# AgamChopra/TorchRegister

Hardware: AMD Instinct MI355X
Metric: registration iterations/sec (3D 256^3 fp32, affine+NCC) (higher is better)
Workload: dtype f32; 1 GPU; 3D 256^3 fp32 affine+NCC, 8 independent pairs per GPU (BASELINE.json configs[3] share of one GPU), ADAM on theta; pairs_per_gpu=8, pairs_total=8, loss=NCC(alpha=100), optimizer=adam, preconditioning=100 untimed iterations before the warm-up (clock settling); value_cold has none, parallelism=1 x independent shards, no collective

## Files before the change

### include/trx.h

```cpp
#ifndef TRX_H
#define TRX_H

#include <stddef.h>
#include <stdint.h>

#ifdef __cplusplus
extern "C" {
#endif

#define TRX_VERSION 240
#define TRX_PSTRIDE 12

typedef enum {
    TRX_OK = 0,
    TRX_ERR_ARG = -1,
    TRX_ERR_NDIM = -2,
    TRX_ERR_WORKSPACE = -3,
    TRX_ERR_HIP = -4,
    TRX_ERR_CAPACITY = -5
} trx_status;

#define TRX_FLAG_GATHER_PATH 1u
#define TRX_FLAG_SINGLE_GEOM 2u
#define TRX_FLAG_TWO_PASS_FLOW 4u
// ... 8 lines not shown
#define TRX_FLAG_WALK_DOWN 8192u
#define TRX_FLAG_NO_PINGPONG 16384u
#define TRX_FLAG_NO_ZS_FLAT 4096u
#define TRX_FLAG_ONE_KERNEL 32768u
#define TRX_FLAG_NO_CARRY 65536u
#define TRX_FLAG_NO_ROT_DEEP_TILE 16u

typedef struct {
    const float *moving;
    const float *target;
    size_t moving_stride;
    size_t target_stride;
    int ndim, B, D, H, W;
    const float *xn, *yn, *zn;
    unsigned flags;
} trx_volumes;

typedef struct {
    float w_mse, w_ncc, ncc_alpha, w_ssd, ssd_alpha;
} trx_loss_cfg;

typedef enum { TRX_OPT_SGD = 0, TRX_OPT_ADAM = 1 } trx_opt_kind;
typedef struct {
    int kind;
    float lr, beta1, beta2, eps;
} trx_opt_cfg;

typedef enum { TRX_PARAM_AFFINE = 0, TRX_PARAM_RIGID = 1 } trx_param_mode;

typedef struct {
    int mode;
    float *param;
    float *theta;
    float *adam_m;
    float *adam_v;
    float *best_theta;
    float *best_loss;
    int *best_idx;
    float *losses;
    int losses_capacity;
    int *step;
    float *grad;
} trx_affine_state;

int trx_version(void);
const char *trx_status_string(int status);

size_t trx_affine_workspace_bytes(const trx_volumes *vol );

size_t trx_affine_workspace_rows_offset(const trx_volumes *vol );

int trx_affine_near_identity(const trx_volumes *vol , const float *theta_host);

int trx_affine_step(const trx_volumes *vol, const trx_loss_cfg *loss, const trx_opt_cfg *opt,
                    const trx_affine_state *st, void *workspace, size_t workspace_bytes, void *stream);

int trx_affine_accumulate(const trx_volumes *vol, const float *theta, void *workspace, size_t workspace_bytes, void *stream);

int trx_affine_run(const trx_volumes *vol, const trx_loss_cfg *loss, const trx_opt_cfg *opt,
                   const trx_affine_state *st, int iters, void *workspace, size_t workspace_bytes, void *stream);

int trx_affine_loss(const trx_volumes *vol, const trx_loss_cfg *loss, const float *theta, float *terms,
                    void *workspace, size_t workspace_bytes, void *stream);

int trx_affine_warp(const trx_volumes *vol, const float *theta, int channels, float *out, void *stream);

int trx_affine_warp_backward(const trx_volumes *vol, const float *theta, int channels, const float *grad_out,
                             float *dtheta, void *workspace, size_t workspace_bytes, void *stream);

int trx_affine_warp_lattice(const trx_volumes *vol, const float *theta, const int *iz, int nz, const int *iy, int ny, const int *ix, int nx,
                            float *out, void *stream);
int trx_affine_warp_lattice_backward(const trx_volumes *vol, const float *theta, const int *iz, int nz, const int *iy, int ny, const int *ix,
                                     int nx, const float *grad_out, float *dtheta, void *workspace, size_t workspace_bytes, void *stream);

int trx_theta_chain(const float *pose, const float *dtheta, int ndim, int B, float *theta_out, float *dpose_out, void *stream);

typedef struct {
    float *flow;
    float *flow_tmp;
    float *adam_m;
    float *adam_v;
    float *losses;
    int losses_capacity;
    int *step;
    float smooth_weight;
    float stop_crit;
    int *stopped;
    float *flow_last;
} trx_flow_state;

size_t trx_flow_workspace_bytes(const trx_volumes *vol);

int trx_flow_warp(const trx_volumes *vol, const float *flow, int channels, float *out, void *stream);

int trx_flow_step(const trx_volumes *vol, const trx_loss_cfg *loss, const trx_opt_cfg *opt,
                  const trx_flow_state *st, void *workspace, size_t workspace_bytes, void *stream);
int trx_flow_run(const trx_volumes *vol, const trx_loss_cfg *loss, const trx_opt_cfg *opt,
                 const trx_flow_state *st, int iters, void *workspace, size_t workspace_bytes, void *stream);

int trx_flow_loss_grad(const trx_volumes *vol, const trx_loss_cfg *loss, const float *flow, float *terms,
                       float *dflow, void *workspace, size_t workspace_bytes, void *stream);

int trx_flow_slab_moments(const trx_volumes *vol, int z_offset, int D_full, const float *flow, int smooth, const float *halo_hi, double *moments,
                          void *workspace, size_t workspace_bytes, void *stream);
int trx_flow_slab_update(const trx_volumes *vol, int z_offset, int D_full, const trx_loss_cfg *loss, const trx_opt_cfg *opt,
                         const trx_flow_state *st, const double *global_moments, const float *halo_lo, const float *halo_hi,
// ... 64 lines not shown
```

### torchregister_amd/_lib.py

```python
import ctypes
import os

import torch

_HERE = os.path.dirname(os.path.abspath(__file__))
LIB_PATH = os.path.join(_HERE, "lib", "libtrx.so")

PSTRIDE = 12
OPT_SGD, OPT_ADAM = 0, 1
PARAM_AFFINE, PARAM_RIGID = 0, 1
FLAG_GATHER_PATH, FLAG_SINGLE_GEOM, FLAG_TWO_PASS_FLOW, FLAG_DEEP_TILE, FLAG_NO_ROT_DEEP_TILE, FLAG_NO_ZSTREAM, FLAG_ZSTREAM, FLAG_NEAREST, FLAG_SAVE_LAST = 1, 2, 4, 8, 16, 32, 64, 128, 256
FLAG_NO_EFT, FLAG_EFT = 512, 1024
FLAG_WALK_DOWN, FLAG_NO_PINGPONG = 8192, 16384
FLAG_NO_ZS_FLAT = 4096
FLAG_ONE_KERNEL = 32768
FLAG_NO_CARRY = 65536
FLAG_ZS_FUSED = 2048

c_float_p = ctypes.POINTER(ctypes.c_float)
c_int_p = ctypes.POINTER(ctypes.c_int)


class TrxError(RuntimeError):
    pass


class Volumes(ctypes.Structure):
    _fields_ = [("moving", ctypes.c_void_p), ("target", ctypes.c_void_p),
                ("moving_stride", ctypes.c_size_t), ("target_stride", ctypes.c_size_t),
                ("ndim", ctypes.c_int), ("B", ctypes.c_int), ("D", ctypes.c_int), ("H", ctypes.c_int), ("W", ctypes.c_int),
                ("xn", ctypes.c_void_p), ("yn", ctypes.c_void_p), ("zn", ctypes.c_void_p), ("flags", ctypes.c_uint)]


class LossCfg(ctypes.Structure):
    _fields_ = [("w_mse", ctypes.c_float), ("w_ncc", ctypes.c_float), ("ncc_alpha", ctypes.c_float),
                ("w_ssd", ctypes.c_float), ("ssd_alpha", ctypes.c_float)]


class OptCfg(ctypes.Structure):
    _fields_ = [("kind", ctypes.c_int), ("lr", ctypes.c_float), ("beta1", ctypes.c_float), ("beta2", ctypes.c_float),
                ("eps", ctypes.c_float)]


class AffineState(ctypes.Structure):
    _fields_ = [("mode", ctypes.c_int), ("param", ctypes.c_void_p), ("theta", ctypes.c_void_p),
                ("adam_m", ctypes.c_void_p), ("adam_v", ctypes.c_void_p), ("best_theta", ctypes.c_void_p),
                ("best_loss", ctypes.c_void_p), ("best_idx", ctypes.c_void_p), ("losses", ctypes.c_void_p),
                ("losses_capacity", ctypes.c_int), ("step", ctypes.c_void_p), ("grad", ctypes.c_void_p)]


class FlowState(ctypes.Structure):
    _fields_ = [("flow", ctypes.c_void_p), ("flow_tmp", ctypes.c_void_p), ("adam_m", ctypes.c_void_p),
                ("adam_v", ctypes.c_void_p), ("losses", ctypes.c_void_p), ("losses_capacity", ctypes.c_int),
                ("step", ctypes.c_void_p), ("smooth_weight", ctypes.c_float), ("stop_crit", ctypes.c_float),
                ("stopped", ctypes.c_void_p), ("flow_last", ctypes.c_void_p)]


_P = ctypes.c_void_p
SIGNATURES = {
    "trx_version": (ctypes.c_int, []),
    "trx_status_string": (ctypes.c_char_p, [ctypes.c_int]),
    "trx_affine_workspace_bytes": (ctypes.c_size_t, [ctypes.POINTER(Volumes)]),
    "trx_affine_workspace_rows_offset": (ctypes.c_size_t, [ctypes.POINTER(Volumes)]),
    "trx_affine_near_identity": (ctypes.c_int, [ctypes.POINTER(Volumes), _P]),
    "trx_affine_step": (ctypes.c_int, [ctypes.POINTER(Volumes), ctypes.POINTER(LossCfg), ctypes.POINTER(OptCfg),
                                       ctypes.POINTER(AffineState), _P, ctypes.c_size_t, _P]),
    "trx_affine_accumulate": (ctypes.c_int, [ctypes.POINTER(Volumes), _P, _P, ctypes.c_size_t, _P]),
    "trx_affine_run": (ctypes.c_int, [ctypes.POINTER(Volumes), ctypes.POINTER(LossCfg), ctypes.POINTER(OptCfg),
                                      ctypes.POINTER(AffineState), ctypes.c_int, _P, ctypes.c_size_t, _P]),
    "trx_affine_loss": (ctypes.c_int, [ctypes.POINTER(Volumes), ctypes.POINTER(LossCfg), _P, _P, _P, ctypes.c_size_t, _P]),
    "trx_affine_warp": (ctypes.c_int, [ctypes.POINTER(Volumes), _P, ctypes.c_int, _P, _P]),
    "trx_affine_warp_backward": (ctypes.c_int, [ctypes.POINTER(Volumes), _P, ctypes.c_int, _P, _P, _P, ctypes.c_size_t, _P]),
    "trx_theta_chain": (ctypes.c_int, [_P, _P, ctypes.c_int, ctypes.c_int, _P, _P, _P]),
    "trx_affine_warp_lattice": (ctypes.c_int, [ctypes.POINTER(Volumes), _P, _P, ctypes.c_int, _P, ctypes.c_int, _P, ctypes.c_int, _P, _P]),
    "trx_affine_warp_lattice_backward": (ctypes.c_int, [ctypes.POINTER(Volumes), _P, _P, ctypes.c_int, _P, ctypes.c_int, _P, ctypes.c_int, _P, _P, _P,
                                                        ctypes.c_size_t, _P]),
    "trx_flow_workspace_bytes": (ctypes.c_size_t, [ctypes.POINTER(Volumes)]),
    "trx_flow_warp": (ctypes.c_int, [ctypes.POINTER(Volumes), _P, ctypes.c_int, _P, _P]),
    "trx_flow_step": (ctypes.c_int, [ctypes.POINTER(Volumes), ctypes.POINTER(LossCfg), ctypes.POINTER(OptCfg),
                                     ctypes.POINTER(FlowState), _P, ctypes.c_size_t, _P]),
    "trx_flow_run": (ctypes.c_int, [ctypes.POINTER(Volumes), ctypes.POINTER(LossCfg), ctypes.POINTER(OptCfg),
                                    ctypes.POINTER(FlowState), ctypes.c_int, _P, ctypes.c_size_t, _P]),
    "trx_flow_slab_moments": (ctypes.c_int, [ctypes.POINTER(Volumes), ctypes.c_int, ctypes.c_int, _P, ctypes.c_int, _P, _P, _P, ctypes.c_size_t, _P]),
    "trx_flow_slab_boundary_smooth": (ctypes.c_int, [ctypes.POINTER(Volumes), _P, _P, _P, _P]),
    "trx_peer_signal": (ctypes.c_int, [_P, ctypes.c_uint, _P]),
    "trx_peer_wait": (ctypes.c_int, [_P, ctypes.c_uint, ctypes.c_uint, _P, _P]),
    "trx_peer_publish": (ctypes.c_int, [_P, _P, _P, ctypes.c_int, ctypes.c_uint, _P]),
    "trx_peer_gather": (ctypes.c_int, [_P, _P, ctypes.c_int, ctypes.c_uint, ctypes.c_uint, _P, _P, _P]),
    "trx_peer_alloc": (ctypes.c_int, [ctypes.c_size_t, ctypes.POINTER(ctypes.c_void_p)]),
    "trx_peer_free": (ctypes.c_int, [_P]),
    "trx_peer_export": (ctypes.c_int, [_P, _P]),
    "trx_peer_import": (ctypes.c_int, [_P, ctypes.POINTER(ctypes.c_void_p)]),
    "trx_peer_close": (ctypes.c_int, [_P]),
    "trx_flow_slab_update": (ctypes.c_int, [ctypes.POINTER(Volumes), ctypes.c_int, ctypes.c_int, ctypes.POINTER(LossCfg),
                                            ctypes.POINTER(OptCfg), ctypes.POINTER(FlowState), _P, _P, _P, _P, ctypes.c_size_t, _P]),
    "trx_flow_slab_update_fused": (ctypes.c_int, [ctypes.POINTER(Volumes), ctypes.c_int, ctypes.c_int, ctypes.POINTER(LossCfg),
                                                  ctypes.POINTER(OptCfg), ctypes.POINTER(FlowState), _P, _P, ctypes.c_size_t, _P]),
    "trx_flow_slab_moments_ready": (ctypes.c_int, [ctypes.POINTER(Volumes), ctypes.c_int, ctypes.c_int, _P, _P, ctypes.c_size_t, _P]),
    "trx_flow_loss_grad": (ctypes.c_int, [ctypes.POINTER(Volumes), ctypes.POINTER(LossCfg), _P, _P, _P, _P, ctypes.c_size_t, _P]),
    "trx_flow_warp_backward": (ctypes.c_int, [ctypes.POINTER(Volumes), _P, ctypes.c_int, _P, _P, _P]),
    "trx_kde_workspace_bytes": (ctypes.c_size_t, [ctypes.c_int, ctypes.c_long, ctypes.c_int]),
    "trx_kde_pdf": (ctypes.c_int, [_P, _P, ctypes.c_int, ctypes.c_long, ctypes.c_int, ctypes.c_float, _P, _P, ctypes.c_size_t, _P]),
    "trx_kde_pdf_backward": (ctypes.c_int, [_P, _P, _P, ctypes.c_int, ctypes.c_long, ctypes.c_int, ctypes.c_float, _P, _P]),
    "trx_kde_series_workspace_bytes": (ctypes.c_size_t, [ctypes.c_int, ctypes.c_long, ctypes.c_int]),
    "trx_kde_pdf_series": (ctypes.c_int, [_P, _P, ctypes.c_int, ctypes.c_long, ctypes.c_int, ctypes.c_float, ctypes.c_double, _P, _P, ctypes.c_size_t, _P]),
    "trx_kde_pdf_series_backward": (ctypes.c_int, [_P, _P, _P, ctypes.c_int, ctypes.c_long, ctypes.c_int, ctypes.c_float, ctypes.c_double, _P, _P,
                                                   ctypes.c_size_t, _P]),
    "trx_kde_pdf_series_cached": (ctypes.c_int, [_P, _P, ctypes.c_int, ctypes.c_int, ctypes.c_long, ctypes.c_int, ctypes.c_float, ctypes.c_double, _P, _P]),
    "trx_nmi_from_pdfs_pooled": (ctypes.c_int, [_P, _P, _P, ctypes.c_int, ctypes.c_int, ctypes.c_float, _P, _P, _P, _P, _P]),
    "trx_nmi_lattice_lines": (ctypes.c_int, [ctypes.POINTER(Volumes), _P, _P, ctypes.c_int, _P, ctypes.c_int, _P, ctypes.c_int, _P, _P, ctypes.c_int,
                                             ctypes.c_int, _P, _P, _P, ctypes.c_size_t, _P]),
    "trx_nmi_loop_update": (ctypes.c_int, [ctypes.c_int, _P, _P, _P, _P, ctypes.c_float, _P, ctypes.c_int, _P, _P, _P, _P, _P]),
    "trx_nmi_from_pdfs": (ctypes.c_int, [_P, _P, _P, ctypes.c_int, ctypes.c_int, ctypes.c_float, _P, _P, _P, _P, _P, _P, _P]),
    "trx_flow_lncc_workspace_bytes": (ctypes.c_size_t, [ctypes.POINTER(Volumes)]),
    "trx_flow_lncc_run": (ctypes.c_int, [ctypes.POINTER(Volumes), ctypes.c_int, ctypes.c_float, ctypes.c_float, ctypes.POINTER(OptCfg),
                                         ctypes.POINTER(FlowState), ctypes.c_int, _P, ctypes.c_size_t, _P]),
    "trx_lncc_workspace_bytes": (ctypes.c_size_t, [ctypes.c_int] * 5),
# ... 37 lines not shown
```

### torchregister_amd/csrc/affine.hip

```cpp
#ifdef TRX_DEV
#include <cstdlib>
#endif
#include "trx_dev.h"

#include "trx_common.h"

namespace trx {

struct AffineGeom {
    int TX, TY, logTX, RPT, nxseg, nychunk, nblk;
};

static AffineGeom affine_geom(const trx_volumes &v, int target_blocks_total)
{
    AffineGeom g;
    int tx = 16, l = 4;
    while (tx < v.W && tx < TRX_BLOCK) { tx <<= 1; l++; }
    g.TX = tx; g.logTX = l; g.TY = TRX_BLOCK / tx;
    g.nxseg = (v.W + tx - 1) / tx;
    long rows = (long)v.D * v.H * g.nxseg * v.B;
    long rpt = rows / ((long)g.TY * target_blocks_total);
    if (rpt < 1) rpt = 1;
    if (rpt > 64) rpt = 64;
    g.RPT = (int)rpt;
// ... 2061 lines not shown
    p.zs_first = p.flat && p.zg.blocks_per_pair > 0 && !(v.flags & TRX_FLAG_ZS_FUSED);
    p.one_kernel = p.zs_first && (v.flags & TRX_FLAG_ONE_KERNEL);
    const bool two_body = !p.flat && p.td.blocks_per_pair == 0 && p.trd.blocks_per_pair == 0 && p.zg.blocks_per_pair == 0 && p.eft == 0;
    p.dual = p.zs_first ? kBehindZs : !two_body ? kFiveBody : carry ? kCarry : kTwoBody;
    return p;
}

struct AffineWs {
    size_t rows, off_tab, off_rows_used, off_part2, off_rows_used2, off_carry, bytes;
};
static AffineWs affine_ws(const trx_volumes &v)
{
    AffineWs w;
    AffineGeom g = affine_geom(v, kTargetBlocks);
    w.rows = (size_t)g.nblk;
    if (v.ndim == 3) w.rows = max(w.rows, (size_t)f1_rows(f1_candidates(v)));
    w.off_tab = ((size_t)v.B * w.rows * np_full(3) * sizeof(float) + 255) & ~(size_t)255;
    w.off_rows_used = w.off_tab + (((size_t)(v.W + v.H + v.D) * sizeof(float) + 255) & ~(size_t)255);
    const size_t notes = ((size_t)(v.B + 11) * sizeof(int) + 255) & ~(size_t)255;
    w.off_part2 = w.off_rows_used + notes;
    w.off_rows_used2 = w.off_part2 + (v.ndim == 3 ? w.off_tab : 0);
    w.off_carry = w.off_rows_used2 + (v.ndim == 3 ? notes : 0);
    w.bytes = w.off_carry + (v.ndim == 3 ? (((size_t)2 * v.B * kCarryStride * sizeof(float) + 255) & ~(size_t)255) : 0);
    return w;
}

extern "C" size_t trx_affine_workspace_bytes(const trx_volumes *vol)
{
    if (check_vol(vol, false) != TRX_OK) return 0;
    return affine_ws(*vol).bytes;
}

extern "C" size_t trx_affine_workspace_rows_offset(const trx_volumes *vol)
{
    if (check_vol(vol, false) != TRX_OK) return 0;
    return affine_ws(*vol).off_rows_used;
}

extern "C" int trx_affine_near_identity(const trx_volumes *vol, const float *theta_host)
{
    if (check_vol(vol, false) != TRX_OK || !theta_host || vol->ndim != 3) return 0;
    const F1Plan p = f1_plan(*vol, persistent_blocks(), true, false);
    if (p.zg.blocks_per_pair == 0) return 0;
    const float fD = (float)vol->D, fH = (float)vol->H, fW = (float)vol->W;
    for (int b = 0; b < vol->B; b++) {
        const float *th = theta_host + (size_t)b * TRX_PSTRIDE;
        if (zs_nsub<ZS64>(th, fD, fH, fW, p.zg.planes_per_seg) > 0) continue;
        if (p.zgf.blocks_per_pair > 0 && zs_nsub<ZSF>(th, fD, fH, fW, p.zgf.planes_per_seg) > 0) continue;
        return 0;
    }
    return 1;
}

static bool use_tile_path(const trx_volumes *vol) { return vol->ndim == 3 && !(vol->flags & TRX_FLAG_GATHER_PATH); }

struct CarryLaunch {
    int parity;
    CarryKArgs args;
    bool used;
    float *partials_out;
};

template <int MODE>
static int launch_accum(const trx_volumes *vol, const float *theta, const AffineGeom &g, int channels, size_t chan_stride,
                        float *partials, hipStream_t s)
{
    dim3 grid(g.nblk, vol->B), block(TRX_BLOCK);
    if (vol->ndim == 3)
        hipLaunchKernelGGL((affine_accum_kernel<3, MODE>), grid, block, 0, s, *vol, theta, g, channels, chan_stride, partials);
    else
        hipLaunchKernelGGL((affine_accum_kernel<2, MODE>), grid, block, 0, s, *vol, theta, g, channels, chan_stride, partials);
    TRX_CHECK_LAUNCH();
    return TRX_OK;
}

template <int MODE>
static void launch_dual(const F1Plan &p, hipStream_t s, const trx_volumes &v, const float *theta, int channels, float *out, int *rows_used = nullptr,
                        const CarryKArgs *carry = nullptr)
{
    const dim3 grid = p.flat ? dim3(p.slots, 1) : dim3(p.rows, v.B * channels);
    const int zero_surplus = rows_used == nullptr, rows_stride = p.flat ? p.rows : 0;
    auto launch = [&](auto which, auto... carry_args) {
        hipLaunchKernelGGL((affine_tile_dual_kernel<MODE, decltype(which)::value>), grid, dim3(512), 0, s, v, theta, p.ta, p.tr, channels, out, zero_surplus, p.td, p.trd, p.zg,
                           rows_used, rows_stride, p.eft, carry_args...);
    };
    if constexpr (MODE == 0 || MODE == 4)
        if (p.dual == kCarry) return launch(Which<kCarry>{}, *carry);
    if constexpr (MODE == 0 || MODE == 1 || MODE == 4)
        if (p.dual == kBehindZs) return launch(Which<kBehindZs>{});
    p.dual == kTwoBody ? launch(Which<kTwoBody>{}) : launch(Which<kFiveBody>{});
}

template <int MODE>
static int launch_f1(const trx_volumes *vol, const float *theta, float *partials, int *nblk, hipStream_t s, const int **rows_used = nullptr, CarryLaunch *cl = nullptr)
{
    if (rows_used) *rows_used = nullptr;
    if (cl) cl->used = false;
    if (!use_tile_path(vol)) {
        if constexpr (MODE == 4) return TRX_ERR_ARG;
        else {
            AffineGeom g = affine_geom(*vol, kTargetBlocks);
            *nblk = g.nblk;
            return launch_accum<MODE>(vol, theta, g, 1, 0, partials, s);
        }
    }
    trx_volumes v = *vol;
// ... 353 lines not shown
```

### torchregister_amd/csrc/affine_zstream.h

```cpp

#ifndef TRX_ZS_DBG
#define TRX_ZS_DBG 0
#endif
#ifndef TRX_ZS_MIN_WAVES
#define TRX_ZS_MIN_WAVES 4
#endif
#ifndef TRX_ZS_PRIO_BIT
#define TRX_ZS_PRIO_BIT 14
#endif
#ifndef TRX_ZS_STAMP
#define TRX_ZS_STAMP 0
#endif
#if TRX_ZS_STAMP
__device__ unsigned long long trx_zs_stamps[512 * 8 * 8];
#endif

struct ZAcc {
    f2 Axy[3], Bxy[3], ABz[3], M01, M23;
    float M4;
};
__device__ __forceinline__ unsigned long long sgpr_pair(float lo, float hi)
{
    const unsigned l = (unsigned)__builtin_amdgcn_readfirstlane(__float_as_int(lo)), h = (unsigned)__builtin_amdgcn_readfirstlane(__float_as_int(hi));
    return ((unsigned long long)h << 32) | l;
}
__device__ __forceinline__ void zs_lerp_accumulate(f2 r00, f2 r01, f2 r10, f2 r11, float tx, float ty, float tz, float yv, float yn, unsigned long long yn2, ZAcc &a)
{
    const f2 dz0 = r10 - r00, dz1 = r11 - r01;
    const f2 z0 = dz0 * tz + r00, z1 = dz1 * tz + r01;
    const f2 dy = z1 - z0;
    const f2 vv = dy * ty + z0;
    const f2 dzy = (dz1 - dz0) * ty + dz0;
    f2 yw, gxy, gz2;
    yw.x = yv;
    gxy.x = vv.y - vv.x;
    asm("v_fma_f32 %0, %1, %2, %3" : "=v"(yw.y) : "v"(tx), "v"(gxy.x), "v"(vv.x));
    asm("v_fma_f32 %0, %1, %2, %3" : "=v"(gxy.y) : "v"(tx), "v"(dy.y - dy.x), "v"(dy.x));
    asm("v_fma_f32 %0, %1, %2, %3" : "=v"(gz2.x) : "v"(tx), "v"(dzy.y - dzy.x), "v"(dzy.x));
    gz2.y = yn * gz2.x;
    f2 ygxy;
    asm("v_pk_mul_f32 %0, %1, %2" : "=v"(ygxy) : "v"(gxy), "s"(yn2));
    a.M01 += yw;
    a.M23 = yw * yw + a.M23;
    a.M4 = fmaf(yw.x, yw.y, a.M4);
    a.Axy[0] += gxy; a.Bxy[0] += ygxy; a.ABz[0] += gz2;
    a.Axy[1] = gxy * yw.x + a.Axy[1]; a.Bxy[1] = ygxy * yw.x + a.Bxy[1]; a.ABz[1] = gz2 * yw.x + a.ABz[1];
    a.Axy[2] = gxy * yw.y + a.Axy[2]; a.Bxy[2] = ygxy * yw.y + a.Bxy[2]; a.ABz[2] = gz2 * yw.y + a.ABz[2];
}

template <int TX_, int TY_, int NZ_, int BW_, int BH_>
struct ZCfg {
    static constexpr int TX = TX_, TY = TY_, NZ = NZ_, BW = BW_, BH = BH_;
    static constexpr int Threads = 512, Waves = 8;
    static constexpr int XW = TX / 64, RG = Waves / XW, R = TY / RG;
    static constexpr int BW4 = BW / 4, PlaneSlots = BH * BW4;
    static constexpr int LPP = (PlaneSlots + 15) / 16;
    static constexpr int PlaneFloats = BW * BH, PlaneBytes = PlaneFloats * 4;
    static constexpr int RingFloats = NZ * PlaneFloats;
    static constexpr int Lead = 1;
    static constexpr int Span = NZ - Lead;
    static constexpr int ReduceScratch = Waves * 16 * 65 + Waves * 16;
    static constexpr int Alloc = (RingFloats + 4 > ReduceScratch) ? RingFloats + 4 : ReduceScratch;
    static_assert(TX % 64 == 0 && Waves % XW == 0 && TY % RG == 0 && BW % 4 == 0 && LPP <= 64 && NZ >= 4 && NZ <= 8 && Span <= 7, "geometry");
};
using ZSF = ZCfg<64, 16, 8, 80, 30>;
using ZS64 = ZCfg<64, 32, 7, 72, 40>;

struct ZGeom {
    int ntx, nty, nzseg, planes_per_seg, blocks_per_pair;
};

template <class C>
static ZGeom zs_geom(const trx_volumes &v)
{
    ZGeom g;
    g.ntx = v.W / C::TX; g.nty = v.H / C::TY;
    const long cols = (long)v.B * g.ntx * g.nty;
    int nseg = cols >= 512 ? 1 : (int)((512 + cols - 1) / cols);
    const int cap = v.D / 32 > 1 ? v.D / 32 : 1;
    if (nseg > cap) nseg = cap;
    g.planes_per_seg = (v.D + nseg - 1) / nseg;
    g.nzseg = (v.D + g.planes_per_seg - 1) / g.planes_per_seg;
    g.blocks_per_pair = g.ntx * g.nty * g.nzseg;
    return g;
}

template <class C>
static bool zs_shape_ok(const trx_volumes &v)
{
    if (v.ndim != 3 || v.W % C::TX || v.H % C::TY || v.D < 8) return false;
    return (size_t)v.D * v.H * v.W < ((size_t)1 << 29);
}

template <class C>
__host__ __device__ __forceinline__ bool zs_fits_len(const float *__restrict__ th, float fD, float fH, float fW, int len)
{
    const float ex = (float)(C::TX - 1), ey = (float)(C::TY - 1), ez = (float)(len - 1);
    const float sx = fabsf(th[0]) * ex + fabsf(th[1] * fW / fH) * ey + fabsf(th[2] * fW / fD) * ez;
    const float sy = fabsf(th[4] * fH / fW) * ex + fabsf(th[5]) * ey + fabsf(th[6] * fH / fD) * ez;
    const float sz = fabsf(th[8] * fD / fW) * ex + fabsf(th[9] * fD / fH) * ey + fabsf(th[10] - 1.0f) * ez;
    return (sx <= (float)C::BW - 6.3f) && (sy <= (float)C::BH - 3.3f) && (sz <= (float)C::Span - 3.3f);
}
template <class C>
__host__ __device__ __forceinline__ int zs_nsub(const float *__restrict__ th, float fD, float fH, float fW, int planes_per_seg)
{
    if (zs_fits_len<C>(th, fD, fH, fW, planes_per_seg)) return 1;
    if (planes_per_seg >= 64 && zs_fits_len<C>(th, fD, fH, fW, (planes_per_seg + 1) / 2)) return 2;
    if (planes_per_seg >= 128 && zs_fits_len<C>(th, fD, fH, fW, (planes_per_seg + 3) / 4)) return 4;
    if (planes_per_seg >= 128 && zs_fits_len<C>(th, fD, fH, fW, (planes_per_seg + 7) / 8)) return 8;
    return 0;
}

#pragma clang diagnostic push
#pragma clang diagnostic ignored "-Winline-asm"
#pragma clang diagnostic ignored "-Wint-to-pointer-cast"
template <int MODE, class C>
__device__ __forceinline__ void zstream_body(const trx_volumes &vol, const float *__restrict__ theta, const ZGeom &zg, float *__restrict__ partials,
                                             float *ring, const int bx, const int by, int rows_per_pair, const int wave_in, const int second_slot = 0)
{
    const int walk_down = __builtin_amdgcn_readfirstlane((int)(vol.flags & TRX_FLAG_WALK_DOWN));
    const int dir = walk_down ? -1 : 1;
    const bool down = walk_down != 0;
    static_assert(MODE == 0 || MODE == 1 || MODE == 4, "step kernels and the moments pass");
    constexpr int NQ = (MODE == 0) ? 3 : (MODE == 4 ? 1 : 0);
    constexpr int NP = (MODE == 0) ? np_full(3) : (MODE == 4 ? kNpMse : 5);
    constexpr bool kGrad = MODE != 1;
    constexpr int R = C::R;
    const int b = by;
    const int D = vol.D, H = vol.H, W = vol.W;
    const float *__restrict__ th = uni_ptr(theta + (size_t)b * TRX_PSTRIDE);
    const float *__restrict__ mov = uni_ptr(vol.moving + (size_t)b * vol.moving_stride);
    const float *__restrict__ tgt = uni_ptr(vol.target + (size_t)b * vol.target_stride);
    const float *__restrict__ xtab = uni_ptr(vol.xn), *__restrict__ ytab = uni_ptr(vol.yn), *__restrict__ ztab = uni_ptr(vol.zn);
    const int lane = trx_lane_id();
    const int wave = __builtin_amdgcn_readfirstlane(wave_in);
    const int tid = wave * 64 + lane;
    const float fW = (float)W, fH = (float)H, fD = (float)D;
    const float hW = 0.5f * fW, hH = 0.5f * fH, hD = 0.5f * fD;
    const float t00 = th[0], t01 = th[1], t02 = th[2], t03 = th[3];
    const float t10 = th[4], t11 = th[5], t12 = th[6], t13 = th[7];
    const float t20 = th[8], t21 = th[9], t22 = th[10], t23 = th[11];

    const int ncol = zg.ntx * zg.nty, nblk = zg.blocks_per_pair;
    int lb = bx;
    if ((nblk & 7) == 0) lb = (bx & 7) * (nblk >> 3) + (bx >> 3);
    const int zseg = lb / ncol, col = lb - zseg * ncol;
    const int X0 = (col % zg.ntx) * C::TX, Y0 = (col / zg.ntx) * C::TY;
    const int zb0 = zseg * zg.planes_per_seg, ze0 = min(zb0 + zg.planes_per_seg, D);
    const int nsub = max(1, __builtin_amdgcn_readfirstlane(zs_nsub<C>(th, fD, fH, fW, zg.planes_per_seg)));
    const int sublen = (zg.planes_per_seg + nsub - 1) / nsub;

    const int xw = wave % C::XW, rg = wave / C::XW;
    const int x = X0 + xw * 64 + lane, yrow0 = Y0 + rg * R;
    const float xn = xtab[x];
    const float cx = unnorm<3>(xn, fW) + hW * fmaf(t00 - 1.0f, xn, t03);
    const float cy = hH * fmaf(t10, xn, t13);
    const float cz = hD * fmaf(t20, xn, t23);
    const float kxz = uni(hW * t02), kyz = uni(hH * t12), kzz = uni(hD * (t22 - 1.0f));
    float yn_r[R], sx_r[R], ey_r[R], sz_r[R];
#pragma unroll
    for (int j = 0; j < R; j++) {
        const float yn = ytab[yrow0 + j];
        yn_r[j] = uni(yn);
        sx_r[j] = uni((hW * t01) * yn);
        ey_r[j] = uni(unnorm<3>(yn, fH) + (hH * (t11 - 1.0f)) * yn);
        sz_r[j] = uni((hD * t21) * yn);
    }
    constexpr bool kV2 = MODE == 0 && (R % 2 == 0);
    unsigned long long sx2[(R + 1) / 2], ey2[(R + 1) / 2], sz2[(R + 1) / 2], yn2[R];
    if constexpr (kV2) {
#pragma unroll
        for (int k = 0; k < R / 2; k++) {
            sx2[k] = sgpr_pair(sx_r[2 * k], sx_r[2 * k + 1]);
            ey2[k] = sgpr_pair(ey_r[2 * k], ey_r[2 * k + 1]);
            sz2[k] = sgpr_pair(sz_r[2 * k], sz_r[2 * k + 1]);
        }
#pragma unroll
        for (int j = 0; j < R; j++) yn2[j] = sgpr_pair(yn_r[j], yn_r[j]);
    }
    auto coord = [&](int xi, int yi, int zi, float &ix, float &iy, float &iz) {
        const float a = xtab[xi], bb = ytab[yi], c = ztab[zi];
        ix = unnorm<3>(a, fW) + hW * fmaf(t00 - 1.0f, a, fmaf(t01, bb, fmaf(t02, c, t03)));
        iy = unnorm<3>(bb, fH) + hH * fmaf(t10, a, fmaf(t11 - 1.0f, bb, fmaf(t12, c, t13)));
        iz = unnorm<3>(c, fD) + hD * fmaf(t20, a, fmaf(t21, bb, fmaf(t22 - 1.0f, c, t23)));
    };

    const unsigned ring_lds = (unsigned)(uintptr_t)ring;
    const unsigned dummy_lds = ring_lds + C::RingFloats * 4u;
    const unsigned pl0 = ring_lds + (unsigned)(wave * C::LPP * 16), pl1 = ring_lds + (unsigned)((wave + 8) * C::LPP * 16);
    const size_t plane_bytes = (size_t)H * W * 4;
    const unsigned toffb = (unsigned)((yrow0 * W) + x) * 4u;
    int ys_s, ps_s;
    asm("s_mov_b32 %0, %1" : "=s"(ys_s) : "i"(C::BW * 4));
    asm("s_mov_b32 %0, %1" : "=s"(ps_s) : "i"(C::PlaneBytes));
    typedef const __attribute__((address_space(3))) f2u *lds_f2;

    F1Acc acc;
#pragma unroll
    for (int q = 0; q < 3; q++)
#pragma unroll
        for (int c = 0; c < 3; c++) acc.AB[q][c] = (f2)(0.f);
    acc.M01 = acc.M23 = (f2)(0.f);
    acc.M4 = 0.f;
    ZAcc acc2;
    f2 Uxy[3];
    float Uz[3];
#pragma unroll
    for (int q = 0; q < 3; q++) {
        acc2.Axy[q] = acc2.Bxy[q] = acc2.ABz[q] = Uxy[q] = (f2)(0.f);
        Uz[q] = 0.f;
    }
    acc2.M01 = acc2.M23 = (f2)(0.f);
    acc2.M4 = 0.f;
    float U[3][3];
#pragma unroll
    for (int q = 0; q < 3; q++)
#pragma unroll
        for (int c = 0; c < 3; c++) U[q][c] = 0.f;
    bool ok = true;
#if TRX_ZS_STAMP
    unsigned long long stamp_sum[6] = {0, 0, 0, 0, 0, 0};
    const unsigned long long stamp_t0 = __builtin_amdgcn_s_memtime(), stamp_r0 = __builtin_amdgcn_s_memrealtime();
#endif

    for (int si = 0; si < nsub; si++) {
        const int sub = down ? nsub - 1 - si : si;
        const int zb = zb0 + sub * sublen, ze = min(zb + sublen, ze0);
        if (zb >= ze) continue;
        const int nsteps = ze - zb, last = nsteps - 1;
        const int zf = down ? ze - 1 : zb, zl = down ? zb : ze - 1;
        float mnx = 1e30f, mxx = -1e30f, mny = 1e30f, mxy = -1e30f, mnz0 = 1e30f, mxz0 = -1e30f, mnz1 = 1e30f, mxz1 = -1e30f;
#pragma unroll
        for (int k = 0; k < 8; k++) {
            float ix, iy, iz;
            coord(X0 + ((k & 1) ? C::TX - 1 : 0), Y0 + ((k & 2) ? C::TY - 1 : 0), (k & 4) ? zl : zf, ix, iy, iz);
            mnx = fminf(mnx, ix); mxx = fmaxf(mxx, ix); mny = fminf(mny, iy); mxy = fmaxf(mxy, iy);
            if (k & 4) { mnz1 = fminf(mnz1, iz); mxz1 = fmaxf(mxz1, iz); } else { mnz0 = fminf(mnz0, iz); mxz0 = fmaxf(mxz0, iz); }
        }
        const float slack = 0.05f;
        bool fits = (fabsf(mnx) < 1.0e6f) && (fabsf(mxx) < 1.0e6f) && (fabsf(mny) < 1.0e6f) && (fabsf(mxy) < 1.0e6f) && (fabsf(mnz0) < 1.0e6f) &&
                    (fabsf(mxz0) < 1.0e6f) && (fabsf(mnz1) < 1.0e6f) && (fabsf(mxz1) < 1.0e6f);
        int ox = 0, oy = 0, pbase = 0, need_rows = 0, need_c4 = 0;
        if (fits) {
            ox = (int)floorf(mnx - slack) & ~3;
            oy = (int)floorf(mny - slack);
            const int hx = (int)floorf(mxx + slack) + 1, hy = (int)floorf(mxy + slack) + 1;
            need_rows = hy - oy; need_c4 = (hx - ox) >> 2;
            const int hi0 = (int)floorf(mxz0 + slack) + 1, hi1 = (int)floorf(mxz1 + slack) + 1;
            const int lo0 = (int)floorf(mnz0 - slack), lo1 = (int)floorf(mnz1 - slack);
            if (!down) {
                pbase = max(hi0, hi1 - last);
                fits = (hx <= ox + C::BW - 1) && (hy <= oy + C::BH - 1) && (lo0 >= pbase - (C::Span - 1)) && (lo1 >= pbase + last - (C::Span - 1));
            } else {
                pbase = min(lo0, lo1 + last);
                fits = (hx <= ox + C::BW - 1) && (hy <= oy + C::BH - 1) && (hi0 <= pbase + (C::Span - 1)) && (hi1 <= pbase - last + (C::Span - 1));
            }
        }
        ox = __builtin_amdgcn_readfirstlane(ox); oy = __builtin_amdgcn_readfirstlane(oy); pbase = __builtin_amdgcn_readfirstlane(pbase);
        need_rows = __builtin_amdgcn_readfirstlane(need_rows); need_c4 = __builtin_amdgcn_readfirstlane(need_c4);
        if (!__builtin_amdgcn_readfirstlane((int)fits)) { ok = false; break; }

        for (int i = tid; i < C::RingFloats / 4; i += C::Threads) reinterpret_cast<float4 *>(ring)[i] = make_float4(0.f, 0.f, 0.f, 0.f);
        unsigned long long mk[2];
        unsigned voff[2];
        bool pvalid[2];
#pragma unroll
        for (int k = 0; k < 2; k++) {
            const int q = wave + 8 * k;
            const int slot = q * C::LPP + lane;
            const bool valid = (lane < C::LPP) && (slot < C::PlaneSlots);
            const int row = slot / C::BW4, c4 = slot - row * C::BW4;
            const int gy = oy + row, gx = ox + 4 * c4;
            const bool inb = valid && (row <= need_rows) && (c4 <= need_c4) && (gy >= 0) && (gy < H) && (gx >= 0) && (gx + 4 <= W);
            mk[k] = __builtin_amdgcn_ballot_w64(inb);
            voff[k] = inb ? (unsigned)((row * W + 4 * c4) * 4) : 0u;
            pvalid[k] = valid;
        }
        const bool real0 = mk[0] != 0, real1 = mk[1] != 0;
        const unsigned long long em0 = real0 ? mk[0] : 1ull, em1 = real1 ? mk[1] : 1ull;
        auto dma2 = [&](const char *b0, const char *b1, unsigned l0, unsigned l1, unsigned long long k0, unsigned long long k1) {
            unsigned long long sv;
            unsigned m0s;
            asm volatile("s_mov_b64 %[sv], exec\n\t"
                         "s_mov_b32 %[m0s], m0\n\t"
                         "s_mov_b32 m0, %[l0]\n\t"
                         "s_mov_b64 exec, %[k0]\n\t"
                         "global_load_lds_dwordx4 %[o0], %[b0]" TRX_ZS_RING_POLICY "\n\t"
                         "s_mov_b32 m0, %[l1]\n\t"
                         "s_mov_b64 exec, %[k1]\n\t"
                         "global_load_lds_dwordx4 %[o1], %[b1]" TRX_ZS_RING_POLICY "\n\t"
                         "s_mov_b64 exec, %[sv]\n\t"
                         "s_mov_b32 m0, %[m0s]"
                         : [sv] "=&s"(sv), [m0s] "=&s"(m0s)
                         : [l0] "s"(l0), [l1] "s"(l1), [b0] "s"(b0), [b1] "s"(b1), [o0] "v"(voff[0]), [o1] "v"(voff[1]), [k0] "s"(k0), [k1] "s"(k1)
                         : "memory");
        };
        auto issue_plane = [&](int p, int slot, const char *gb) {
            if (TRX_ZS_DBG & 1) return;
            const unsigned so = (unsigned)slot * (unsigned)C::PlaneBytes;
            const char *mv = reinterpret_cast<const char *>(mov);
            if ((unsigned)p < (unsigned)D) {
                dma2(real0 ? gb : mv, real1 ? gb : mv, real0 ? pl0 + so : dummy_lds, real1 ? pl1 + so : dummy_lds, em0, em1);
            } else {
                dma2(mv, mv, dummy_lds, dummy_lds, 1ull, 1ull);
#pragma unroll
                for (int k = 0; k < 2; k++)
                    if (pvalid[k]) *reinterpret_cast<float4 *>(ring + slot * C::PlaneFloats + ((wave + 8 * k) * C::LPP + lane) * 4) = make_float4(0.f, 0.f, 0.f, 0.f);
            }
        };
        auto plane_ptr = [&](int p) { return reinterpret_cast<const char *>(mov + ((ptrdiff_t)p * H + oy) * W + ox); };
        auto pmod = [&](int p) { const int m = p % C::NZ; return m < 0 ? m + C::NZ : m; };
        auto issue_targets = [&](const float *trow , float (&tv)[R]) {
// ... 61 lines not shown
                asm("v_mad_i32_i24 %0, %1, %2, %3" : "=v"(a1) : "v"(floor_to_int(iy)), "s"(ys_s), "v"(a0));
                asm("v_mad_u32_u24 %0, %1, %2, %3" : "=v"(aA) : "v"(__builtin_amdgcn_perm((unsigned)(tabA >> 32), (unsigned)tabA, sel)), "s"(ps_s), "v"(a1));
                asm("v_mad_u32_u24 %0, %1, %2, %3" : "=v"(aB) : "v"(__builtin_amdgcn_perm((unsigned)(tabB >> 32), (unsigned)tabB, sel)), "s"(ps_s), "v"(a1));
                Fetch f;
                if (TRX_ZS_DBG & 32) {
                    f.r00 = f2{__int_as_float(aA), ix}; f.r01 = f2{iy, __int_as_float(aB)}; f.r10 = f2{iz, ix}; f.r11 = f2{iy, iz};
                } else {
                if (!(TRX_ZS_DBG & 128)) { f.r00 = *(lds_f2)(unsigned)aA; f.r01 = *(lds_f2)(unsigned)(aA + C::BW * 4); }
                f.r10 = *(lds_f2)(unsigned)aB; f.r11 = *(lds_f2)(unsigned)(aB + C::BW * 4);
                if (TRX_ZS_DBG & 128) {
                    f.r00 = f.r10; f.r01 = f.r11;
                    asm volatile("" : "+v"(f.r00.x), "+v"(f.r00.y), "+v"(f.r01.x), "+v"(f.r01.y), "+v"(aA));
                }
                }
                f.fx = __builtin_amdgcn_fractf(ix); f.fy = __builtin_amdgcn_fractf(iy); f.fz = __builtin_amdgcn_fractf(iz);
                return f;
            };
            Fetch cur = fetch(0);
#pragma unroll
            for (int j = 0; j < R; j++) {
                Fetch nxt;
                if (j + 1 < R) nxt = fetch(j + 1);
                if (TRX_ZS_DBG & 64) {
                    const Samp3 sm = lerp3_pairs<kGrad>(cur.r00, cur.r01, cur.r10, cur.r11, cur.fx, cur.fy, cur.fz);
                    acc2.M4 += sm.v + sm.dx + sm.dy + sm.dz + tv[j];
                } else if constexpr (kV2) {
                    zs_lerp_accumulate(cur.r00, cur.r01, cur.r10, cur.r11, cur.fx, cur.fy, cur.fz, tv[j], yn_r[j], yn2[j], acc2);
                } else {
                    const Samp3 sm = lerp3_pairs<kGrad>(cur.r00, cur.r01, cur.r10, cur.r11, cur.fx, cur.fy, cur.fz);
                    f1_accumulate_pk<MODE>(sm, tv[j], yn_r[j], acc);
                }
                if (j + 1 < R) cur = nxt;
            }
            if constexpr (kV2) {
#pragma unroll
                for (int q = 0; q < 3; q++) { Uxy[q] += acc2.Axy[q]; Uz[q] += acc2.ABz[q].x; }
            } else if constexpr (kGrad) {
#pragma unroll
                for (int q = 0; q < (NQ > 0 ? NQ : 1); q++)
#pragma unroll
                    for (int c = 0; c < 3; c++) U[q][c] += acc.AB[q][c].x;
            }
        };

        auto retreat_tables = [&]() {
            mlo = (mlo == 0) ? C::NZ - 1 : mlo - 1;
            tabB = tabA;
            tabA = (tabA << 8) | (unsigned long long)mlo;
            selc += 1u;
        };

        const ptrdiff_t tstep = (ptrdiff_t)dir * H * W, dstep = (ptrdiff_t)dir * (ptrdiff_t)plane_bytes;
        const float *tnext = tgt + (ptrdiff_t)(zf + dir) * H * W;
        const char *dnext = plane_ptr(pbase + dir * C::Lead);
        int dslot = pmod(pbase + dir * C::Lead);
        auto step = [&](int s, float (&use)[R], float (&load)[R]) {
#if TRX_ZS_STAMP
            const unsigned long long st0 = __builtin_amdgcn_s_memtime();
            unsigned long long st1 = st0, st2 = st0;
#endif
            if (((__builtin_amdgcn_s_memtime() >> TRX_ZS_PRIO_BIT) + second_slot) & 1) __builtin_amdgcn_s_setprio(1); else __builtin_amdgcn_s_setprio(0);
            if (s > 0) {
                if ((s & 63) == 0) {
                    load_ztab(s);
                    asm volatile("s_waitcnt vmcnt(0)" ::: "memory");
                } else if (TRX_ZS_DBG & 16) {
                } else asm volatile("s_waitcnt vmcnt(0)" ::: "memory");
#if TRX_ZS_STAMP
                st1 = __builtin_amdgcn_s_memtime();
#endif
                if (!(TRX_ZS_DBG & 8)) __syncthreads();
#if TRX_ZS_STAMP
                st2 = __builtin_amdgcn_s_memtime();
#endif
                if (down) retreat_tables(); else advance_tables();
            }
#pragma unroll
            for (int j = 0; j < R; j++) asm volatile("" : "+v"(use[j]));
            if (s + 1 <= last) { issue_targets(tnext, load); tnext += tstep; }
            if (s + C::Lead <= last) {
                issue_plane(pbase + dir * (s + C::Lead), dslot, dnext);
                dnext += dstep;
                dslot += dir;
                dslot = (dslot == C::NZ) ? 0 : (dslot < 0 ? C::NZ - 1 : dslot);
            }
#if TRX_ZS_STAMP
            const unsigned long long st3 = __builtin_amdgcn_s_memtime();
#endif
            gather_plane(s, use);
#if TRX_ZS_STAMP
            const unsigned long long st4 = __builtin_amdgcn_s_memtime();
            stamp_sum[0] += st1 - st0; stamp_sum[1] += st2 - st1; stamp_sum[2] += st3 - st2; stamp_sum[3] += st4 - st3; stamp_sum[5] += 1;
#endif
        };

        float tvA[R], tvB[R];
#pragma unroll
        for (int j = 0; j < R; j++) tvA[j] = tvB[j] = 0.f;
        load_ztab(0);
        set_tables(down ? pbase : pbase - (C::Span - 1));
        __syncthreads();
        {
            const int ahead = min(last, C::Lead - 1);
            const int pa = down ? pbase - ahead : pbase - (C::Span - 1), pb = down ? pbase + (C::Span - 1) : pbase + ahead;
            for (int p = pa; p <= pb; p++) issue_plane(p, pmod(p), plane_ptr(p));
        }
        issue_targets(tgt + (size_t)zf * H * W, tvA);
        asm volatile("s_waitcnt vmcnt(0)" ::: "memory");
        __syncthreads();
        int s = 0;
        while (s < nsteps) {
            step(s, tvA, tvB);
            s++;
            if (s >= nsteps) break;
            step(s, tvB, tvA);
            s++;
        }
        __syncthreads();
    }

    __builtin_amdgcn_s_setprio(0);
    if (!ok) {
        if (tid < NP) partials[((size_t)by * rows_per_pair + bx) * NP + tid] = __builtin_nanf("");
        return;
    }
    float vals[NP];
    int o = 0;
    if constexpr (kV2) {
        vals[0] = acc2.M01.x; vals[1] = acc2.M01.y; vals[2] = acc2.M23.x; vals[3] = acc2.M23.y; vals[4] = acc2.M4;
        o = 5;
    } else if constexpr (MODE == 4) {
        vals[0] = acc.M4;
        o = 1;
    } else {
        vals[0] = acc.M01.x; vals[1] = acc.M01.y; vals[2] = acc.M23.x; vals[3] = acc.M23.y; vals[4] = acc.M4;
        o = 5;
    }
// ... 50 lines not shown
```

Baseline: 26670 pair-iterations/s.

## Let z-stream window follow the z-scale drift instead of widening for zoom

```diff
diff --git a/include/trx.h b/include/trx.h
--- a/include/trx.h
+++ b/include/trx.h
@@ -84,6 +84,8 @@
 
 int trx_affine_near_identity(const trx_volumes *vol , const float *theta_host);
 
+int trx_affine_zs_windows(const trx_volumes *vol , const float *theta_host, int *out);
+
 int trx_affine_step(const trx_volumes *vol, const trx_loss_cfg *loss, const trx_opt_cfg *opt,
                     const trx_affine_state *st, void *workspace, size_t workspace_bytes, void *stream);
 
diff --git a/torchregister_amd/_lib.py b/torchregister_amd/_lib.py
--- a/torchregister_amd/_lib.py
+++ b/torchregister_amd/_lib.py
@@ -63,6 +63,7 @@
     "trx_affine_workspace_bytes": (ctypes.c_size_t, [ctypes.POINTER(Volumes)]),
     "trx_affine_workspace_rows_offset": (ctypes.c_size_t, [ctypes.POINTER(Volumes)]),
     "trx_affine_near_identity": (ctypes.c_int, [ctypes.POINTER(Volumes), _P]),
+    "trx_affine_zs_windows": (ctypes.c_int, [ctypes.POINTER(Volumes), _P, _P]),
     "trx_affine_step": (ctypes.c_int, [ctypes.POINTER(Volumes), ctypes.POINTER(LossCfg), ctypes.POINTER(OptCfg),
                                        ctypes.POINTER(AffineState), _P, ctypes.c_size_t, _P]),
     "trx_affine_accumulate": (ctypes.c_int, [ctypes.POINTER(Volumes), _P, _P, ctypes.c_size_t, _P]),
diff --git a/torchregister_amd/csrc/affine.hip b/torchregister_amd/csrc/affine.hip
--- a/torchregister_amd/csrc/affine.hip
+++ b/torchregister_amd/csrc/affine.hip
@@ -2137,6 +2137,17 @@
     return 1;
 }
 
+extern "C" int trx_affine_zs_windows(const trx_volumes *vol, const float *theta_host, int *out)
+{
+    if (check_vol(vol, false) != TRX_OK || !theta_host || !out || vol->ndim != 3) return 0;
+    const F1Plan p = f1_plan(*vol, persistent_blocks(), true, false);
+    const float fD = (float)vol->D, fH = (float)vol->H, fW = (float)vol->W;
+    for (int b = 0; b < vol->B; b++)
+        out[b] = p.zg.blocks_per_pair > 0 ? zs_nsub<ZS64>(theta_host + (size_t)b * TRX_PSTRIDE, fD, fH, fW, p.zg.planes_per_seg) : 0;
+    out[vol->B] = p.zg.blocks_per_pair > 0 ? p.zg.planes_per_seg : 0;
+    return p.zg.blocks_per_pair > 0;
+}
+
 static bool use_tile_path(const trx_volumes *vol) { return vol->ndim == 3 && !(vol->flags & TRX_FLAG_GATHER_PATH); }
 
 struct CarryLaunch {
diff --git a/torchregister_amd/csrc/affine_zstream.h b/torchregister_amd/csrc/affine_zstream.h
--- a/torchregister_amd/csrc/affine_zstream.h
+++ b/torchregister_amd/csrc/affine_zstream.h
@@ -64,7 +64,7 @@
     static_assert(TX % 64 == 0 && Waves % XW == 0 && TY % RG == 0 && BW % 4 == 0 && LPP <= 64 && NZ >= 4 && NZ <= 8 && Span <= 7, "geometry");
 };
 using ZSF = ZCfg<64, 16, 8, 80, 30>;
-using ZS64 = ZCfg<64, 32, 7, 72, 40>;
+using ZS64 = ZCfg<64, 32, 7, 76, 38>;
 
 struct ZGeom {
     int ntx, nty, nzseg, planes_per_seg, blocks_per_pair;
@@ -92,13 +92,20 @@
     return (size_t)v.D * v.H * v.W < ((size_t)1 << 29);
 }
 
+__host__ __device__ __forceinline__ float zs_follow_cost(float t22) { return t22 > 1.0f ? 2.0f : 1.0f; }
+__host__ __device__ __forceinline__ bool zs_follows(float t22, int len)
+{
+    const float k = fabsf(t22 - 1.0f);
+    return k < 0.5f && k * (float)(len - 1) > zs_follow_cost(t22);
+}
 template <class C>
 __host__ __device__ __forceinline__ bool zs_fits_len(const float *__restrict__ th, float fD, float fH, float fW, int len)
 {
     const float ex = (float)(C::TX - 1), ey = (float)(C::TY - 1), ez = (float)(len - 1);
     const float sx = fabsf(th[0]) * ex + fabsf(th[1] * fW / fH) * ey + fabsf(th[2] * fW / fD) * ez;
     const float sy = fabsf(th[4] * fH / fW) * ex + fabsf(th[5]) * ey + fabsf(th[6] * fH / fD) * ez;
-    const float sz = fabsf(th[8] * fD / fW) * ex + fabsf(th[9] * fD / fH) * ey + fabsf(th[10] - 1.0f) * ez;
+    const float zoom = zs_follows(th[10], len) ? zs_follow_cost(th[10]) : fabsf(th[10] - 1.0f) * ez;
+    const float sz = fabsf(th[8] * fD / fW) * ex + fabsf(th[9] * fD / fH) * ey + zoom;
     return (sx <= (float)C::BW - 6.3f) && (sy <= (float)C::BH - 3.3f) && (sz <= (float)C::Span - 3.3f);
 }
 template <class C>
@@ -149,6 +156,15 @@
     const int zb0 = zseg * zg.planes_per_seg, ze0 = min(zb0 + zg.planes_per_seg, D);
     const int nsub = max(1, __builtin_amdgcn_readfirstlane(zs_nsub<C>(th, fD, fH, fW, zg.planes_per_seg)));
     const int sublen = (zg.planes_per_seg + nsub - 1) / nsub;
+    static_assert(C::Lead == 1, "the planes a step stages are the ones the next step's window gains");
+    const bool follow = __builtin_amdgcn_readfirstlane((int)zs_follows(t22, sublen)) != 0;
+    const bool zoom_in = __builtin_amdgcn_readfirstlane((int)(t22 > 1.0f)) != 0;
+    const unsigned lead_k = follow ? (unsigned)__builtin_amdgcn_readfirstlane(min(32767, max(1, (int)(fabsf(t22 - 1.0f) * 65536.0f + 0.5f)))) : 0u;
+    const unsigned lead_inc = zoom_in ? lead_k : (65536u - lead_k) & 0xffffu;
+    const float lead_rate = zoom_in ? 1.0f + (float)lead_k * (1.0f / 65536.0f) : 1.0f - (float)lead_k * (1.0f / 65536.0f);
+    const int win = follow && zoom_in ? C::Span - 1 : C::Span;
+    unsigned lead = 0;
+    auto lead_planes = [&]() { return 1 - (int)((lead >> 15) & 1u) + (int)(lead < (lead << 16)); };
 
     const int xw = wave % C::XW, rg = wave / C::XW;
     const int x = X0 + xw * 64 + lane, yrow0 = Y0 + rg * R;
@@ -248,7 +264,15 @@
             need_rows = hy - oy; need_c4 = (hx - ox) >> 2;
             const int hi0 = (int)floorf(mxz0 + slack) + 1, hi1 = (int)floorf(mxz1 + slack) + 1;
             const int lo0 = (int)floorf(mnz0 - slack), lo1 = (int)floorf(mnz1 - slack);
-            if (!down) {
+            if (follow) {
+                const float fr0 = down ? -mnz0 : mxz0, fr1 = down ? -mnz1 : mxz1, bk0 = down ? -mxz0 : mnz0, bk1 = down ? -mxz1 : mnz1;
+                const float run = (float)last * lead_rate;
+                const float pc0 = fmaxf(fr0, fr1 - run) + slack + 2.0f, pf = floorf(pc0);
+                pbase = dir * (int)pf;
+                lead = (min(65535u, (unsigned)((pc0 - pf) * 65536.0f)) << 16) | lead_inc;
+                const float reach = (float)(win - 1) - slack - 1.0f;
+                fits = (hx <= ox + C::BW - 1) && (hy <= oy + C::BH - 1) && (bk0 + reach >= pc0) && (bk1 + reach >= pc0 + run);
+            } else if (!down) {
                 pbase = max(hi0, hi1 - last);
                 fits = (hx <= ox + C::BW - 1) && (hy <= oy + C::BH - 1) && (lo0 >= pbase - (C::Span - 1)) && (lo1 >= pbase + last - (C::Span - 1));
             } else {
@@ -258,6 +282,7 @@
         }
         ox = __builtin_amdgcn_readfirstlane(ox); oy = __builtin_amdgcn_readfirstlane(oy); pbase = __builtin_amdgcn_readfirstlane(pbase);
         need_rows = __builtin_amdgcn_readfirstlane(need_rows); need_c4 = __builtin_amdgcn_readfirstlane(need_c4);
+        lead = (unsigned)__builtin_amdgcn_readfirstlane((int)lead);
         if (!__builtin_amdgcn_readfirstlane((int)fits)) { ok = false; break; }
 
         for (int i = tid; i < C::RingFloats / 4; i += C::Threads) reinterpret_cast<float4 *>(ring)[i] = make_float4(0.f, 0.f, 0.f, 0.f);
@@ -425,8 +450,9 @@
 
         const ptrdiff_t tstep = (ptrdiff_t)dir * H * W, dstep = (ptrdiff_t)dir * (ptrdiff_t)plane_bytes;
         const float *tnext = tgt + (ptrdiff_t)(zf + dir) * H * W;
-        const char *dnext = plane_ptr(pbase + dir * C::Lead);
-        int dslot = pmod(pbase + dir * C::Lead);
+        int pnext = pbase + dir;
+        const char *dnext = plane_ptr(pnext);
+        int dslot = pmod(pnext);
         auto step = [&](int s, float (&use)[R], float (&load)[R]) {
 #if TRX_ZS_STAMP
             const unsigned long long st0 = __builtin_amdgcn_s_memtime();
@@ -446,16 +472,30 @@
 #if TRX_ZS_STAMP
                 st2 = __builtin_amdgcn_s_memtime();
 #endif
-                if (down) retreat_tables(); else advance_tables();
+                if (lead == 0) {
+                    if (down) retreat_tables(); else advance_tables();
+                } else {
+                    for (int k = lead_planes(); k > 0; k--) {
+                        if (down) retreat_tables(); else advance_tables();
+                    }
+                }
             }
 #pragma unroll
             for (int j = 0; j < R; j++) asm volatile("" : "+v"(use[j]));
             if (s + 1 <= last) { issue_targets(tnext, load); tnext += tstep; }
             if (s + C::Lead <= last) {
-                issue_plane(pbase + dir * (s + C::Lead), dslot, dnext);
-                dnext += dstep;
-                dslot += dir;
-                dslot = (dslot == C::NZ) ? 0 : (dslot < 0 ? C::NZ - 1 : dslot);
+                auto stage = [&]() {
+                    issue_plane(pnext, dslot, dnext);
+                    pnext += dir;
+                    dnext += dstep;
+                    dslot += dir;
+                    dslot = (dslot == C::NZ) ? 0 : (dslot < 0 ? C::NZ - 1 : dslot);
+                };
+                if (lead == 0) stage();
+                else {
+                    lead += lead << 16;
+                    for (int k = lead_planes(); k > 0; k--) stage();
+                }
             }
 #if TRX_ZS_STAMP
             const unsigned long long st3 = __builtin_amdgcn_s_memtime();
```

Measured after the change: 24630 pair-iterations/s. 7.6% lower.
